# nmonette/TO-UED

Measured on AMD Instinct MI355X. Metric: agent-env-steps/sec (inner rollout) at num_agents=512; meta-updates/sec, higher is better.
Workload: dtype f32; 1 GPU; C2 LPG meta-gradient env_mode=tabular num_agents=512 num_mini_batches=1 W=64 T=20 K=5 score_function=random; num_agents=512, agents_per_gpu=512, env_workers=64, train_rollout_len=20, num_agent_updates=5, parallelism=dp1 (agent axis)

## Files before the change

### to-ued_amd/csrc/gru.hip

```cpp
#include <stdlib.h>
#include <string.h>
#include <algorithm>
#include "common.h"

extern "C" size_t toued_wgrad_workspace_floats(int ra, int rb, long K);
extern "C" int toued_wgrad(int ra, int rb, long K, const float* A, long lda, const float* B, long ldb, float* C,
                           float* work, size_t work_floats, hipStream_t stream);
extern "C" int toued_wgrad_ldc(int ra, int rb, long K, const float* A, long lda, const float* B, long ldb, float* C,
                               int ldc, float* work, size_t work_floats, hipStream_t stream);
extern "C" size_t toued_rowsum_workspace_floats(int ra, long K);
extern "C" int toued_rowsum_into(int ra, long K, const float* A, long lda, float* C, int ldc, float* work,
                                 size_t work_floats, hipStream_t stream);

typedef float floatx16 __attribute__((ext_vector_type(16)));
typedef float floatx4 __attribute__((ext_vector_type(4)));

#define HU 256
#define RB 32
#define LDH 33
#define NAUG 8
#define KQF 33
#define NTILE_F 32

struct EtaOff {
// ... 1211 lines not shown
    }
    __syncthreads();
    float dhn_r[NT][16];
    const float* wil = wi34 + 32 * wave + 4 * hi;
#pragma unroll
    for (int h = 0; h < NT; ++h) {
      floatx16 hacc;
#pragma unroll
      for (int q = 0; q < 16; ++q) hacc[q] = 0.0f;
#pragma unroll
      for (int kk = 0; kk < 5; ++kk) {
        const int o = 2 * kk + hi;
        hacc = mfma32(wA[kk], o < 9 ? hv[o * RBT + RB * h + col] : 0.0f, hacc);
      }
      const unsigned vq = (unsigned)((((long)(32 * wave + 4 * hi + (col & 3))) * p.M + r0 + RB * h + (col & 28)) * 4);
      float dx3 = 0.0f, dx4 = 0.0f;
#pragma unroll
      for (int g4 = 0; g4 < 4; ++g4) {
        const unsigned so = (unsigned)(((long)8 * g4 * p.M + ctr) * 4);
        float v_hin[4], v_r[4], v_z[4], v_n[4], v_hn[4];
        ld4(rs_hin, vq, so, v_hin);
        ld4(rs_r, vq, so, v_r);
        ld4(rs_z, vq, so, v_z);
        ld4(rs_n, vq, so, v_n);
        ld4(rs_hn, vq, so, v_hn);
        quad_transpose(v_hin, lane);
        quad_transpose(v_r, lane);
        quad_transpose(v_z, lane);
        quad_transpose(v_n, lane);
        quad_transpose(v_hn, lane);
        float* o_rh = v_hin; float* o_dr = v_r; float* o_dz = v_z; float* o_dhn = v_n; float* o_dn = v_hn;
#pragma unroll
        for (int j = 0; j < 4; ++j) {
          const int q = 4 * g4 + j;
          const float hin = v_hin[j], rg = v_r[j], zg = v_z[j], ng = v_n[j], hn = v_hn[j];
          const float hout = (1.0f - zg) * ng + zg * hin;
          const float d = dh[h][q] + (hout > 0.0f ? hacc[q] : 0.0f);
          const float dn_ = d * (1.0f - zg);
          const float dz = d * (hin - ng);
          const float dnp = dn_ * (1.0f - ng * ng);
          const float dhn = dnp * rg;
          const float drp = dnp * hn * rg * (1.0f - rg);
          const float dzp = dz * zg * (1.0f - zg);
          dh[h][q] = d * zg;
          const int lo = (32 * wave + 4 * hi + qunit(q)) * LDT + RB * h + col;
          dgT[lo] = drp;
          dgT[HU * LDT + lo] = dzp;
          dhn_r[h][q] = dhn;
          o_rh[j] = fmaxf(hout, 0.0f); o_dr[j] = drp; o_dz[j] = dzp; o_dhn[j] = dhn; o_dn[j] = dnp;
          const int qu = qunit(q);
          dx3 += drp * wil[0 * HU + qu] + dzp * wil[1 * HU + qu] + dnp * wil[2 * HU + qu];
          dx4 += drp * wil[3 * HU + qu] + dzp * wil[4 * HU + qu] + dnp * wil[5 * HU + qu];
        }
        {
          const unsigned vb = (unsigned)(((long)(32 * wave + 4 * hi) * p.M + r0 + RB * h + col) * 4);
#pragma unroll
          for (int j = 0; j < 4; ++j) {
            const unsigned so1 = (unsigned)(((long)qunit(4 * g4 + j) * p.M + ctr) * 4);
            st_u(rs_rh, vb, so1, o_rh[j]);
            st_u(rs_dg[3], vb, so1, o_dn[j]);
          }
        }
      }
      dxp[((2 * wave + hi) * 2 + 0) * RBT + RB * h + col] = dx3;
      dxp[((2 * wave + hi) * 2 + 1) * RBT + RB * h + col] = dx4;
    }
    floatx16 acc[NT];
#pragma unroll
    for (int h = 0; h < NT; ++h)
#pragma unroll
      for (int q = 0; q < 16; ++q) acc[h][q] = 0.0f;
#pragma unroll 1
    for (int g = 0; g < 3; ++g) {
      if (g == 2) {
        __syncthreads();
#pragma unroll
        for (int h = 0; h < NT; ++h) {
          float* dgl = dgT + (32 * wave + 4 * hi) * LDT + RB * h + col;
#pragma unroll
          for (int q = 0; q < 16; ++q) dgl[qunit(q) * LDT] = dhn_r[h][q];
        }
      }
      if (g != 1) __syncthreads();
      if (g == 0) {
        store_gate_lds<NT>(dgT, rs_dg[0], p.M, ctr + r0, wave, lane);
        store_gate_lds<NT>(dgT + HU * LDT, rs_dg[1], p.M, ctr + r0, wave, lane);
      } else if (g == 2) {
        store_gate_lds<NT>(dgT, rs_dg[2], p.M, ctr + r0, wave, lane);
      }
      const float* dgs = dgT + (g == 1 ? HU * LDT : 0);
      float4 an = Ab[((wave * 3 + g) * 32 + 0) * 64];
#pragma unroll 2
      for (int kq = 0; kq < 32; ++kq) {
        const float4 av = an;
        if (kq + 1 < 32) an = Ab[((wave * 3 + g) * 32 + kq + 1) * 64];
#pragma unroll
        for (int e = 0; e < 4; ++e) {
          const float x = e == 0 ? av.x : e == 1 ? av.y : e == 2 ? av.z : av.w;
#pragma unroll
          for (int h = 0; h < NT; ++h) {
            const float b = dgs[(2 * (4 * kq + e) + hi) * LDT + RB * h + col];
            acc[h] = mfma32(x, b, acc[h]);
          }
        }
      }
    }
    __syncthreads();
    if (tid < RBT) {
      float s3 = 0.0f, s4 = 0.0f;
      for (int gq = 0; gq < NGRP; ++gq) { s3 += dxp[(gq * 2 + 0) * RBT + tid]; s4 += dxp[(gq * 2 + 1) * RBT + tid]; }
      p.dX3[ctr + r0 + tid] = s3;
      p.dX4[ctr + r0 + tid] = s4;
    }
#pragma unroll
    for (int h = 0; h < NT; ++h) {
      const bool dn = done[((size_t)a_[h] * T + t) * W + w_[h]] != 0;
#pragma unroll
      for (int q = 0; q < 16; ++q) dh[h][q] = dn ? 0.0f : dh[h][q] + acc[h][q];
    }
    __syncthreads();
  }
}


#ifdef BWD_STAMPS
__device__ unsigned long long g_bwd_stamps[64 * 32 * 8];
#define BWD_STAMP(ph)                                                                                  \
  do {                                                                                                 \
    if (blockIdx.x < 64 && tid == 0 && t < 32)                                                         \
      g_bwd_stamps[(blockIdx.x * 32 + t) * 8 + (ph)] = __builtin_amdgcn_s_memtime();                   \
  } while (0)
#define BWD_NWS 8
__device__ unsigned long long g_bwd_wstamps[64 * 32 * 8 * BWD_NWS];
__device__ int g_bwd_wsimd[64 * 8];
#define BWD_WSTAMP(ph)                                                                                 \
  do {                                                                                                 \
    if (blockIdx.x < 64 && lane_now() == 0 && t < 32)                                                  \
      g_bwd_wstamps[((blockIdx.x * 32 + t) * 8 + wave) * BWD_NWS + (ph)] = __builtin_amdgcn_s_memtime(); \
  } while (0)
#else
#define BWD_STAMP(ph) do {} while (0)
#define BWD_WSTAMP(ph) do {} while (0)
#endif

#ifndef BWD_MPRIO
#define BWD_MPRIO 0
#endif
#ifndef BWD_TRECOMP
#define BWD_TRECOMP 0
#endif
#ifndef BWD_PK
#define BWD_PK 1
#endif
template <bool SMALL>
__global__ void __launch_bounds__(512, 1) k_gru_bwd6n(BwdArgs p) {
  constexpr int RBT = 2 * RB;
  constexpr int PP = HU + 8;
  __shared__ __attribute__((aligned(16))) __bf16 dgB[3][RBT * PP];
  __shared__ float wi34[2 * 3 * HU];
  __shared__ float hv[9 * RBT];
  __shared__ __attribute__((aligned(8))) float dxp[8 * RBT * 2];
  __shared__ __attribute__((aligned(16))) float wsc[HU];
  __shared__ float rmx[8 * RBT];
  __shared__ float wIs[8 * 4 * 64];
  __shared__ float wAs[8 * 5 * 64];
  __shared__ int dns[RBT];
  __shared__ __attribute__((aligned(16))) float Atab[SMALL ? 32 * 64 : 4];
  __shared__ float hvs[SMALL ? 9 * RBT : 1];
  __shared__ floatx4 accl[SMALL ? 8 * 2 * 64 : 1];
  constexpr int DRP = HU + 4;
  static_assert(RBT * DRP * 4 <= 2 * RBT * PP * 2, "dr staging exceeds image slots 1-2");
  float* drs = reinterpret_cast<float*>(&dgB[1][0]);
  const int tid = threadIdx.x, lane = tid & 63, hi = lane >> 5, col = lane & 31;
  const int wave = __builtin_amdgcn_readfirstlane(tid >> 6);
  const int nb = p.R / RBT;
  const int bid = blockIdx.x + p.wg_base;
  const int k = bid / nb;
  const int r0 = (bid - k * nb) * RBT;
  const int R = p.R, T = p.T, W = p.W;
#ifdef BWD_STAMPS
  if (blockIdx.x < 64 && (tid & 63) == 0)
    g_bwd_wsimd[blockIdx.x * 8 + wave] = __builtin_amdgcn_s_getreg((1 << 11) | (4 << 6) | 4);
#endif
  for (int i = tid; i < 2 * 3 * HU; i += 512) {
    const int f = BWD_PK ? 3 + (i & 1) : 3 + i / (3 * HU), g = BWD_PK ? (i >> 1) / HU : (i / HU) % 3,
              u = BWD_PK ? (i >> 1) % HU : i % HU;
    const int base = g == 0 ? p.o.ir_w : g == 1 ? p.o.iz_w : p.o.in_w;
    wi34[i] = f < p.F ? p.eta[base + f * HU + u] : 0.0f;
  }
  for (int i = tid; i < HU; i += 512) wsc[i] = reinterpret_cast<const float*>(p.A6)[B6_SCALES + i];
  const int F = p.F;
  {
    float wI[4];
    load_win_frags(wI, p.eta, p.o, F, wave, lane);
#pragma unroll
    for (int kk = 0; kk < 4; ++kk) wIs[(wave * 4 + kk) * 64 + lane] = wI[kk];
  }
#pragma unroll
  for (int kk = 0; kk < 5; ++kk) {
    const int o = 2 * kk + hi, u = 32 * wave + col;
    wAs[(wave * 5 + kk) * 64 + lane] = o < 9 ? (o == 0 ? p.eta[p.o.pi_w + u] : p.eta[p.o.y_w + u * 8 + (o - 1)]) : 0.0f;
  }
  float dh[2][16];
#pragma unroll
  for (int h = 0; h < 2; ++h)
#pragma unroll
    for (int q = 0; q < 16; ++q) dh[h][q] = 0.0f;
  if (SMALL) {
    for (int i = tid; i < 9 * RBT; i += 512) hvs[i] = 0.0f;
    for (int i = tid; i < 8 * 2 * 64; i += 512) accl[i] = floatx4{0.0f, 0.0f, 0.0f, 0.0f};
  }
  constexpr bool st_rh = !SMALL, st_dn = !SMALL;
  const __amdgpu_buffer_rsrc_t rs_hin = rsrc_of(p.s_hin), rs_r = rsrc_of(p.s_r), rs_z = rsrc_of(p.s_z),
                               rs_hn = rsrc_of(p.s_hn), rs_rh = rsrc_of(SMALL ? p.s_hin : p.RH);
  const __amdgpu_buffer_rsrc_t rs_x = rsrc_of(p.s_hin + (size_t)HU * p.M);
  const __amdgpu_buffer_rsrc_t rs_dg[4] = {rsrc_of(p.DG), rsrc_of(p.DG + 1L * HU * p.M),
                                           rsrc_of(p.DG + 2L * HU * p.M),
                                           rsrc_of(SMALL ? p.DG : p.DG + 3L * HU * p.M)};
  constexpr bool st_DH = !SMALL;
  const __amdgpu_buffer_rsrc_t rs_yh = rsrc_of(p.y_hat), rs_dyh = rsrc_of(p.d_y_hat), rs_dpi = rsrc_of(p.d_pi_hat),
                               rs_DH = rsrc_of(SMALL ? p.dX3 : p.DH), rs_dx3 = rsrc_of(p.dX3), rs_dx4 = rsrc_of(p.dX4),
                               rs_done = rsrc_of(reinterpret_cast<const float*>(p.done + (long)k * p.done_stride_k));
  auto head_cot = [&](int t) {
    if (tid < RBT) {
      const int tl = lane_now();
      const unsigned vrw = (unsigned)tl * 4;
      int dnv;
      {
        const int rw = r0 + tl, a = rw / W;
        dnv = __builtin_amdgcn_raw_buffer_load_b8(rs_done, (a * T + t) * W + rw - a * W, 0, 0);
      }
      const long o = ((long)k * T + t) * R + r0;
      float yh[8], dy[8], s = 0.0f;
#pragma unroll
      for (int j = 0; j < 8; ++j) {
        const unsigned so = (unsigned)((((long)k * T * 8 + (long)t * 8 + j) * R + r0) * 4);
        yh[j] = ld_u(rs_yh, vrw, so);
        dy[j] = ld_u(rs_dyh, vrw, so);
      }
#pragma unroll
      for (int j = 0; j < 8; ++j) s += yh[j] * dy[j];
      const float dpi = ld_u(rs_dpi, vrw, (unsigned)(o * 4));
      float xr[6];
      if (SMALL) {
#pragma unroll
        for (int f = 0; f < 6; ++f)
          xr[f] = ld_u(rs_x, vrw, (unsigned)(((long)(f < F ? f : 0) * p.M + o) * 4));
      }
      dns[tl] = dnv;
      hv[tl] = dpi;
      if (st_DH) st_u(rs_DH, vrw, (unsigned)(o * 4), dpi);
      float hvv[9];
      hvv[0] = dpi;
#pragma unroll
      for (int j = 0; j < 8; ++j) {
        const float v = yh[j] * (dy[j] - s);
        hv[(j + 1) * RBT + tl] = v;
        hvv[j + 1] = v;
        if (st_DH) st_u(rs_DH, vrw, (unsigned)(((long)(j + 1) * p.M + o) * 4), v);
      }
      if (SMALL) {
        float* at = Atab + (tl >> 1) * 64 + 16 * (tl & 1);
#pragma unroll
        for (int c = 0; c < 4; ++c) {
          if (c >= 2) *reinterpret_cast<float4*>(at + 4 * c) = make_float4(0.0f, 0.0f, 0.0f, 0.0f);
          *reinterpret_cast<float4*>(at + 32 + 4 * c) = make_float4(0.0f, 0.0f, 0.0f, 0.0f);
        }
        at[6] = 0.0f;
        at[7] = 0.0f;
        *reinterpret_cast<float4*>(at) = make_float4(0 < F ? xr[0] : 0.0f, 1 < F ? xr[1] : 0.0f, 2 < F ? xr[2] : 0.0f,
                                                     3 < F ? xr[3] : 0.0f);
        *reinterpret_cast<float2*>(at + 4) = make_float2(4 < F ? xr[4] : 0.0f, 5 < F ? xr[5] : 0.0f);
        at[F] = 1.0f;
#pragma unroll
        for (int o9 = 0; o9 < 9; ++o9) at[32 + F + 1 + o9] = hvv[o9];
#pragma unroll
        for (int o9 = 0; o9 < 9; ++o9) hvs[o9 * RBT + tl] += hvv[o9];
      }
    }
  };
  const __amdgpu_buffer_rsrc_t rs_A = rsrc_of(reinterpret_cast<const float*>(p.A6));
  const unsigned vA = (unsigned)lane * 16;
  floatx16 acc[2];
  auto ldAh = [&](int ks, int g, int q) {
    const u32x4 x = __builtin_amdgcn_raw_buffer_load_b128(rs_A, (int)vA,
                                                          (int)((((ks * 8 + wave) * 3 + g) * 3 + q) * 1024), 0);
    return __builtin_bit_cast(f16x8, x);
  };
#ifndef BWD_RD
#define BWD_RD 4
#endif
#ifndef BWD_SPREAD
#define BWD_SPREAD 0
#endif
  auto dg_vbyte = [&](int ub_, int col_) {
    return SMALL ? (unsigned)(ub_ * 128 + col_ * 4) : (unsigned)(((long)ub_ * p.M + r0 + col_) * 4);
  };
  auto dg_soff = [&](long ctr_, int uq, int h) {
    return SMALL ? (unsigned)((((ctr_ + r0) >> 5) + h) * 32768L + uq * 128)
                 : (unsigned)((((long)uq * p.M + ctr_) * 4) + 128 * h);
  };
  auto store_slot = [&](int gst, long ctr_, int gi, int i, float v) {
    const int s_ = 2 * BWD_RD * gi + i, h = s_ >> 4, e = s_ & 3, g4 = (s_ & 15) >> 2;
    const int ln = lane_now();
    st_u(rs_dg[gst], dg_vbyte(32 * wave + 4 * (ln >> 5), ln & 31), dg_soff(ctr_, e + 8 * g4, h), v);
  };
#ifndef BWD_SPLACE
#define BWD_SPLACE 0
#endif
  static_assert(!BWD_SPLACE || (!BWD_SPREAD && 16 % BWD_RD == 0), "BWD_SPLACE: burst stores, RD dividing 16");
  f16x8 ring[BWD_RD][2];
  auto preload_ring = [&](int g) {
#pragma unroll
    for (int i = 0; i < BWD_RD; ++i)
#pragma unroll
      for (int q = 0; q < 2; ++q) ring[i][q] = ldAh(i, g, q);
  };
  auto contract_h = [&](int g, int sb, int sb1, float (&qv)[32], long ctr_, auto&& pre, bool preloaded, int nextg,
                        auto&& post, auto&& inpass) {
    constexpr int RD = BWD_RD;
    static_assert(!BWD_SPREAD || 16 % RD == 0, "the spread stores: 2 per k-step, 2 RD per ring group");
    f16x8 B[2][2];
    if (!preloaded) preload_ring(g);
    const int ln = lane_now(), bl = (ln & 31) * PP + 8 * (ln >> 5);
    auto ldB = [&](int ks, int h) {
#pragma unroll
      for (int q = 0; q < 2; ++q) B[h][q] = *reinterpret_cast<const f16x8*>(&dgB[q ? sb1 : sb][bl + RB * h * PP + 16 * ks]);
    };
    ldB(0, 0);
    ldB(0, 1);
    auto kstep = [&](int ks, f16x8 (&Ar)[2], bool reload, int gi, int j) {
#pragma unroll
      for (int h = 0; h < 2; ++h) {
        acc[h] = mfma3h(Ar, B[h], acc[h]);
        if (ks + 1 < 16) ldB(ks + 1, h);
        if (BWD_SPREAD && h == 0) {
          store_slot(g, ctr_, gi, 2 * j, qv[2 * j]);
          store_slot(g, ctr_, gi, 2 * j + 1, qv[2 * j + 1]);
        }
      }
      if (reload) {
#pragma unroll
        for (int q = 0; q < 2; ++q) Ar[q] = ldAh(ks + RD, g, q);
      }
      __builtin_amdgcn_sched_barrier(0);
    };
    constexpr int NG = (16 - RD) / RD;
#pragma nounroll
    for (int gi = 0; gi < NG; ++gi) {
#pragma unroll
      for (int j = 0; j < RD; ++j) kstep(gi * RD + j, ring[j], true, gi, j);
      if (BWD_SPREAD) {
#pragma unroll
        for (int i = 0; i < 32 - 2 * RD; ++i) qv[i] = qv[i + 2 * RD];
      }
    }
#pragma unroll
    for (int ks = NG * RD; ks < 16; ++ks) {
      kstep(ks, ring[ks % RD], ks + RD < 16, NG, ks - NG * RD);
      if (ks == 16 - RD) {
        pre();
        __builtin_amdgcn_sched_barrier(0);
      }
      if (BWD_SPLACE && nextg >= 0 && ks >= 16 - RD) {
#pragma unroll
        for (int q = 0; q < 2; ++q) ring[ks % RD][q] = ldAh(ks - (16 - RD), nextg, q);
        __builtin_amdgcn_sched_barrier(0);
      }
      if (ks >= 12) {
        inpass(ks - 12);
        __builtin_amdgcn_sched_barrier(0);
      }
    }
    post();
  };
#ifndef BWD_INPASS
#define BWD_INPASS 0
#endif
#ifndef BWD_TREFILL
#define BWD_TREFILL 0
#endif
  auto put4h = [&](int row, int u0, const float (&v)[4], float sc) {
    f16x4 x0, x1;
    if (BWD_TREFILL == 2) {
#pragma unroll
      for (int e = 0; e < 4; ++e) { x0[e] = (_Float16)0.0f; x1[e] = (_Float16)0.0f; }
    } else {
#pragma unroll
      for (int e = 0; e < 4; ++e) split2h(v[e] * sc, x0, x1, e);
    }
    if (BWD_TREFILL != 1) {
      *reinterpret_cast<f16x4*>(&dgB[0][row * PP + u0]) = x0;
      *reinterpret_cast<f16x4*>(&dgB[1][row * PP + u0]) = x1;
    }
  };
  auto put1h = [&](int slot, int which, int row, int u0, const float (&v)[4], float sc) {
    f16x4 x0, x1;
#pragma unroll
    for (int e = 0; e < 4; ++e) split2h(v[e] * sc, x0, x1, e);
    *reinterpret_cast<f16x4*>(&dgB[slot][row * PP + u0]) = which ? x1 : x0;
  };
  float* priv = reinterpret_cast<float*>(&dgB[0][0]) + 1056 * wave;
  auto small_mfma = [&](int h, int g4, const float (&dnq)[4], const float (&rhq)[4]) {
    const int ln = lane_now(), row = ln & 31, c = 2 * (g4 & 1) + (ln >> 5);
    const int wo = row * 16 + ((c ^ ((row >> 2) & 3)) << 2);
    *reinterpret_cast<float4*>(priv + wo) = make_float4(dnq[0], dnq[1], dnq[2], dnq[3]);
    *reinterpret_cast<float4*>(priv + 544 + wo) = make_float4(rhq[0], rhq[1], rhq[2], rhq[3]);
    if (g4 & 1) {
      const int l2 = lane_now(), kk = l2 >> 4, j = l2 & 15;
      const int rb = (kk >> 1) * 544 + (kk & 1) * 16 + (j & 3);
      floatx4& al = accl[(wave * 2 + (g4 >> 1)) * 64 + l2];
      floatx4 acc = al;
#pragma unroll
      for (int s2 = 0; s2 < 16; ++s2) {
        const float b = priv[rb + 32 * s2 + ((((j >> 2) ^ ((s2 >> 1) & 3))) << 2)];
        const float a = Atab[(16 * h + s2) * 64 + l2];
        acc = __builtin_amdgcn_mfma_f32_16x16x4f32(a, b, acc, 0, 0, 0);
      }
      al = acc;
    }
  };
#ifndef BWD_NR
#define BWD_NR 3
#endif
  constexpr int NR = BWD_NR;
  const int ub = 32 * wave + 4 * hi;
  float vr[NR][4][4];
  auto load_q = [&](long ctr_, int h, int g4, float (&v)[4][4]) {
    const unsigned vq = quad_vbyte(ub, col), sq = quad_soff(ctr_ + r0, h, g4);
    if (HIN_SLAB) ld4(rs_hin, slab_vbyte(ub + (col & 3), col & 28), slab_soff(ctr_ + r0, h, 8 * g4), v[0]);
    else ld4(rs_hin, (unsigned)((((long)(ub + (col & 3))) * p.M + r0 + RB * h + (col & 28)) * 4),
             (unsigned)(((long)8 * g4 * p.M + ctr_) * 4), v[0]);
    if (!BWD_TRECOMP) {
      ld4(rs_r, vq, sq, v[1]);
      ld4(rs_z, vq, sq, v[2]);
      ld4(rs_hn, vq, sq, v[3]);
    }
  };
  float xa[4], xb[4];
  auto load_x = [&](long ctr_, int h, float (&x)[4]) {
#pragma unroll
    for (int kk = 0; kk < 4; ++kk) {
      const int ln = lane_now(), k = 2 * kk + (ln >> 5);
      x[kk] = ld_u(rs_x, (unsigned)((((long)(k < F ? k : 0)) * p.M + RB * h + (ln & 31)) * 4), (unsigned)((ctr_ + r0) * 4));
    }
  };
#ifndef BWD_PF
#define BWD_PF 0
#endif
#ifndef BWD_PFX
#define BWD_PFX 0
#endif
  static_assert(BWD_PF >= 0 && BWD_PF <= NR - 1, "BWD_PF: at most the ring's NR - 1 leading quads");
  auto load_first = [&](long ctr_, bool pre) {
    if (pre == (bool)BWD_PFX) load_x(ctr_, 0, xa);
#pragma unroll
    for (int qi = 0; qi < NR - 1; ++qi)
      if (pre == (qi < BWD_PF)) load_q(ctr_, qi >> 2, qi & 3, vr[qi]);
  };
  if (p.stagger > 0 && blockIdx.x < 256) {
    const int ph = p.stagger_mode == 0 ? (blockIdx.x >> 3) & 1 : p.stagger_mode == 1 ? blockIdx.x & 1 : (blockIdx.x >> 3) & 3;
    for (int i = 0; i < ph * p.stagger; ++i) __builtin_amdgcn_s_sleep(127);
  }
  load_first((long)k * T * R, true);
  for (int t = 0; t < T; ++t) {
    const long ctr = ((long)k * T + t) * R;
    BWD_STAMP(0);
    head_cot(t);
    lds_barrier();
    BWD_STAMP(1);
    BWD_WSTAMP(0);
    floatx16 rc[3][2];
    if (BWD_TRECOMP) {
#pragma unroll
      for (int g = 0; g < 3; ++g)
#pragma unroll
        for (int h = 0; h < 2; ++h)
#pragma unroll
          for (int q = 0; q < 16; ++q) rc[g][h][q] = 0.0f;
      f16x8 Ra0[3][2], Ra1[3][2], Rb[2][2];
      const int ln = lane_now(), bl = (ln & 31) * PP + 8 * (ln >> 5);
      auto ldRB = [&](int ks, int h) {
#pragma unroll
        for (int q = 0; q < 2; ++q) Rb[h][q] = *reinterpret_cast<const f16x8*>(&dgB[q][bl + RB * h * PP + 16 * ks]);
      };
#pragma unroll
      for (int g = 0; g < 3; ++g)
#pragma unroll
        for (int q = 0; q < 2; ++q) {
          Ra0[g][q] = ldAh(0, g, q);
          Ra1[g][q] = ldAh(1, g, q);
        }
      ldRB(0, 0);
      ldRB(0, 1);
      auto rstep = [&](int ks, f16x8 (&Ar)[3][2], bool reload) {
#pragma unroll
        for (int g = 0; g < 3; ++g) {
#pragma unroll
          for (int h = 0; h < 2; ++h) {
            rc[g][h] = mfma3h(Ar[g], Rb[h], rc[g][h]);
            if (g == 2 && ks + 1 < 16) ldRB(ks + 1, h);
          }
          if (reload) {
#pragma unroll
            for (int q = 0; q < 2; ++q) Ar[g][q] = ldAh(ks + 2, g, q);
          }
          __builtin_amdgcn_sched_barrier(0);
        }
      };
#pragma nounroll
      for (int kp = 0; kp < 7; ++kp) {
        rstep(2 * kp, Ra0, true);
        rstep(2 * kp + 1, Ra1, true);
      }
      rstep(14, Ra0, false);
      rstep(15, Ra1, false);
      lds_barrier();
    }
    float dz_r[2][16], dhn_r[2][16];
    auto ubn = [&] { return 32 * wave + 4 * (lane_now() >> 5); };
    auto rown = [&](int h) { return RB * h + (lane_now() & 31); };
    auto st_q = [&](__amdgpu_buffer_rsrc_t rs, int h, int g4, const float (&v)[4]) {
#pragma unroll
      for (int e = 0; e < 4; ++e)
        st_u(rs, (unsigned)(((long)ub * p.M + r0 + RB * h + col) * 4),
             (unsigned)(((long)qunit(4 * g4 + e) * p.M + ctr) * 4), v[e]);
    };
    load_first(ctr, false);
    floatx16 ain;
    floatx16 hacc;
    float dx3 = 0.0f, dx4 = 0.0f;
    float rmr[2] = {0.0f, 0.0f};
#pragma unroll
    for (int qi = 0; qi < 8; ++qi) {
      const int h = qi >> 2, g4 = qi & 3;
      if (BWD_MPRIO == 1) {
        if (((qi + (wave >> 2)) & 1) == 0) __builtin_amdgcn_s_setprio(2); else __builtin_amdgcn_s_setprio(1);
      } else if (BWD_MPRIO == 2 && qi == 0) {
        if (wave >= 4) __builtin_amdgcn_s_setprio(2); else __builtin_amdgcn_s_setprio(1);
      }
      float (&v)[4][4] = vr[qi % NR];
      if (qi + NR - 1 < 8) load_q(ctr, (qi + NR - 1) >> 2, (qi + NR - 1) & 3, vr[(qi + NR - 1) % NR]);
      if (qi == 3) load_x(ctr, 1, xb);
      __builtin_amdgcn_sched_barrier(0);
      if (g4 == 0) {
#pragma unroll
        for (int q = 0; q < 16; ++q) hacc[q] = 0.0f;
#pragma unroll
        for (int kk = 0; kk < 5; ++kk) {
          const int ln = lane_now(), o = 2 * kk + (ln >> 5);
          hacc = mfma32(wAs[(wave * 5 + kk) * 64 + ln], o < 9 ? hv[o * RBT + RB * h + (ln & 31)] : 0.0f, hacc);
        }
        float wI[4];
#pragma unroll
        for (int kk = 0; kk < 4; ++kk) wI[kk] = wIs[(wave * 4 + kk) * 64 + lane];
        ain = gate_ain(wI, F, hi, [&](int k) { return h ? xb[k >> 1] : xa[k >> 1]; });
        dx3 = 0.0f;
        dx4 = 0.0f;
      }
      quad_transpose(v[0], lane);
      const float* wil = wi34 + ubn();
      float drq[4], rhq[4], dnq[4];
      if (BWD_PK) {
        const f2v* wil2 = reinterpret_cast<const f2v*>(wi34) + ubn();
        f2v dx34 = {dx3, dx4};
#pragma unroll
        for (int pp = 0; pp < 2; ++pp) {
          const int j0 = 2 * pp, q0 = 4 * g4 + j0;
          const f2v hin = {v[0][j0], v[0][j0 + 1]}, rg = {v[1][j0], v[1][j0 + 1]}, zg = {v[2][j0], v[2][j0 + 1]},
                    hn = {v[3][j0], v[3][j0 + 1]};
          const f2v ng = {gate_n(ain[q0], rg.x, hn.x), gate_n(ain[q0 + 1], rg.y, hn.y)};
          const f2v omz = 1.0f - zg;
          const f2v hout = omz * ng + zg * hin;
          const f2v hac = {hout.x > 0.0f ? hacc[q0] : 0.0f, hout.y > 0.0f ? hacc[q0 + 1] : 0.0f};
          const f2v d = f2v{dh[h][q0], dh[h][q0 + 1]} + hac;
          const f2v dn_ = d * omz;
          const f2v dz = d * (hin - ng);
          const f2v dnp = dn_ * (1.0f - ng * ng);
          const f2v dhn = dnp * rg;
          const f2v drp = dnp * hn * rg * (1.0f - rg);
          const f2v dzp = dz * zg * omz;
          const f2v dhv = d * zg;
#pragma unroll
          for (int e = 0; e < 2; ++e) {
            const int q = q0 + e, qu = qunit(q);
            dh[h][q] = dhv[e];
            drq[j0 + e] = drp[e];
            dz_r[h][q] = dzp[e];
            dhn_r[h][q] = dhn[e];
            rhq[j0 + e] = fmaxf(hout[e], 0.0f);
            dnq[j0 + e] = dnp[e];
            dx34 += f2v{drp[e], drp[e]} * wil2[0 * HU + qu] + f2v{dzp[e], dzp[e]} * wil2[1 * HU + qu] +
                    f2v{dnp[e], dnp[e]} * wil2[2 * HU + qu];
          }
        }
        dx3 = dx34.x;
        dx4 = dx34.y;
      }
#pragma unroll
      for (int jj = 0; jj < (BWD_PK ? 0 : 4); ++jj) {
        const int q = 4 * g4 + jj;
        const float hin = v[0][jj];
        const float rg = BWD_TRECOMP ? sigm_r(rc[0][h][q] * 0.5f) : v[1][jj];
        const float zg = BWD_TRECOMP ? sigm_r(rc[1][h][q] * 0.5f) : v[2][jj];
        const float hn = BWD_TRECOMP ? rc[2][h][q] * 0.5f : v[3][jj];
        const float ng = gate_n(ain[q], rg, hn);
        const float hout = (1.0f - zg) * ng + zg * hin;
        const float d = dh[h][q] + (hout > 0.0f ? hacc[q] : 0.0f);
        const float dn_ = d * (1.0f - zg);
        const float dz = d * (hin - ng);
        const float dnp = dn_ * (1.0f - ng * ng);
        const float dhn = dnp * rg;
        const float drp = dnp * hn * rg * (1.0f - rg);
        const float dzp = dz * zg * (1.0f - zg);
        dh[h][q] = d * zg;
        drq[jj] = drp;
        dz_r[h][q] = dzp;
        dhn_r[h][q] = dhn;
        const int qu = qunit(q);
        dx3 += drp * wil[0 * HU + qu] + dzp * wil[1 * HU + qu] + dnp * wil[2 * HU + qu];
        dx4 += drp * wil[3 * HU + qu] + dzp * wil[4 * HU + qu] + dnp * wil[5 * HU + qu];
        rhq[jj] = fmaxf(hout, 0.0f);
        dnq[jj] = dnp;
      }
      if (st_rh) st_q(rs_rh, h, g4, rhq);
      if (st_dn) st_q(rs_dg[3], h, g4, dnq);
      if (SMALL) small_mfma(h, g4, dnq, rhq);
      *reinterpret_cast<float4*>(&drs[rown(h) * DRP + ubn() + 8 * g4]) = make_float4(drq[0], drq[1], drq[2], drq[3]);
#pragma unroll
      for (int jj = 0; jj < 4; ++jj) rmr[h] = fmaxf(rmr[h], fabsf(drq[jj]));
      if (g4 == 3) {
        const float f3 = dx3 + __shfl_xor(dx3, 32), f4 = dx4 + __shfl_xor(dx4, 32);
        const int ln = lane_now();
        if (ln < 32) *reinterpret_cast<float2*>(dxp + (wave * RBT + RB * h + ln) * 2) = make_float2(f3, f4);
      }
      __builtin_amdgcn_sched_barrier(0);
    }
    if (BWD_MPRIO) __builtin_amdgcn_s_setprio(0);
    BWD_STAMP(2);
    BWD_WSTAMP(1);
#pragma unroll
    for (int h = 0; h < 2; ++h) {
      float m = rmr[h];
#pragma unroll
      for (int q = 0; q < 16; ++q) m = fmaxf(m, fmaxf(fabsf(dz_r[h][q]), fabsf(dhn_r[h][q])));
      m = fmaxf(m, __shfl_xor(m, 32));
      const int ln = lane_now();
      if (ln < 32) rmx[wave * RBT + RB * h + ln] = m;
    }
    lds_barrier();
    BWD_STAMP(3);
    float bs[2];
#pragma unroll
    for (int h = 0; h < 2; ++h) {
      float m = 0.0f;
      const int cl = lane_now() & 31;
#pragma unroll
      for (int w8 = 0; w8 < 8; ++w8) m = fmaxf(m, rmx[w8 * RBT + RB * h + cl]);
      int sc = 0, ce = 127;
      if (m > 0.0f && m <= 3.0e38f) {
        int e;
        frexpf(m, &e);
        sc = min(40, max(-40, 14 - e));
        ce = min(126, max(-126, 14 - e));
      }
      bs[h] = ldexpf(1.0f, sc);
      if (p.CE && wave == 0 && lane_now() < 32) p.CE[ctr + r0 + rown(h)] = (int8_t)ce;
    }
    auto store_dg = [&](int g, int row, int g4, const float (&v)[4]) {
#pragma unroll
      for (int e = 0; e < 4; ++e)
        st_u(rs_dg[g], dg_vbyte(ub, col), dg_soff(ctr, qunit(4 * g4 + e), row >= RB ? 1 : 0), v[e]);
    };
    float qv[32];
    if (BWD_SPLACE) preload_ring(0);
    {
      f16x4 x1h[2][4];
#pragma unroll
      for (int h = 0; h < 2; ++h)
#pragma unroll
        for (int g4 = 0; g4 < 4; ++g4) {
          const int row = rown(h), un = ubn();
          const float4 v = *reinterpret_cast<const float4*>(&drs[row * DRP + un + 8 * g4]);
          const float v4[4] = {v.x, v.y, v.z, v.w};
          f16x4 x0;
#pragma unroll
          for (int e = 0; e < 4; ++e) split2h(v4[e] * bs[h], x0, x1h[h][g4], e);
          *reinterpret_cast<f16x4*>(&dgB[0][row * PP + un + 8 * g4]) = x0;
          if (BWD_SPREAD) {
#pragma unroll
            for (int e = 0; e < 4; ++e) qv[16 * h + 4 * g4 + e] = v4[e];
          } else {
            store_dg(0, RB * h, g4, v4);
          }
        }
      lds_barrier();
#pragma unroll
      for (int h = 0; h < 2; ++h)
#pragma unroll
        for (int g4 = 0; g4 < 4; ++g4)
          *reinterpret_cast<f16x4*>(&dgB[1][rown(h) * PP + ubn() + 8 * g4]) = x1h[h][g4];
      lds_barrier();
    }
    const int un0 = ubn();
#pragma unroll
    for (int g4 = 0; g4 < 4; ++g4) {
      const float4 w4 = *reinterpret_cast<const float4*>(&wsc[un0 + 8 * g4]);
      const float wv[4] = {w4.x, w4.y, w4.z, w4.w};
#pragma unroll
      for (int h = 0; h < 2; ++h)
#pragma unroll
        for (int e = 0; e < 4; ++e) acc[h][4 * g4 + e] = dh[h][4 * g4 + e] * (wv[e] * bs[h]);
    }
    BWD_STAMP(4);
    BWD_WSTAMP(2);
    auto inpass_put = [&](int j, int slot, const float (&src)[2][16]) {
#pragma unroll
      for (int i = 2 * j; i < 2 * j + 2; ++i) {
        const int h = i >> 2, g4 = i & 3;
        const float v4[4] = {src[h][4 * g4], src[h][4 * g4 + 1], src[h][4 * g4 + 2], src[h][4 * g4 + 3]};
        put1h(slot, 0, rown(h), ubn() + 8 * g4, v4, bs[h]);
      }
    };
    contract_h(0, 0, 1, qv, ctr, [] {}, (bool)BWD_SPLACE, BWD_SPLACE ? 1 : -1, [&] {
      if (BWD_SPLACE) {
#pragma unroll
        for (int h = 0; h < 2; ++h)
#pragma unroll
          for (int g4 = 0; g4 < 4; ++g4) {
            const float v4[4] = {dz_r[h][4 * g4], dz_r[h][4 * g4 + 1], dz_r[h][4 * g4 + 2], dz_r[h][4 * g4 + 3]};
            store_dg(1, RB * h, g4, v4);
          }
      }
    }, [&](int j) {
      if (BWD_INPASS) inpass_put(j, 2, dz_r);
    });
    BWD_WSTAMP(3);
    lds_barrier();
    BWD_WSTAMP(4);
#pragma unroll
    for (int h = 0; h < 2; ++h)
#pragma unroll
      for (int g4 = 0; g4 < 4; ++g4) {
        const float v4[4] = {dz_r[h][4 * g4], dz_r[h][4 * g4 + 1], dz_r[h][4 * g4 + 2], dz_r[h][4 * g4 + 3]};
        if (BWD_INPASS) put1h(0, 1, rown(h), ubn() + 8 * g4, v4, bs[h]);
        else put4h(rown(h), ubn() + 8 * g4, v4, bs[h]);
        if (BWD_SPREAD) {
#pragma unroll
          for (int e = 0; e < 4; ++e) qv[16 * h + 4 * g4 + e] = v4[e];
        } else if (!BWD_SPLACE) {
          store_dg(1, RB * h, g4, v4);
        }
      }
    lds_barrier();
    BWD_STAMP(5);
    BWD_WSTAMP(5);
    contract_h(1, BWD_INPASS ? 2 : 0, BWD_INPASS ? 0 : 1, qv, ctr, [] {}, (bool)BWD_SPLACE, BWD_SPLACE ? 2 : -1, [&] {
      if (BWD_SPLACE) {
#pragma unroll
        for (int h = 0; h < 2; ++h)
#pragma unroll
          for (int g4 = 0; g4 < 4; ++g4) {
            const float v4[4] = {dhn_r[h][4 * g4], dhn_r[h][4 * g4 + 1], dhn_r[h][4 * g4 + 2], dhn_r[h][4 * g4 + 3]};
            store_dg(2, RB * h, g4, v4);
          }
      }
    }, [&](int j) {
      if (BWD_INPASS) inpass_put(j, 1, dhn_r);
    });
    BWD_WSTAMP(6);
    lds_barrier();
    BWD_WSTAMP(7);
#pragma unroll
    for (int h = 0; h < 2; ++h)
#pragma unroll
      for (int g4 = 0; g4 < 4; ++g4) {
        const float v4[4] = {dhn_r[h][4 * g4], dhn_r[h][4 * g4 + 1], dhn_r[h][4 * g4 + 2], dhn_r[h][4 * g4 + 3]};
        if (BWD_INPASS) put1h(2, 1, rown(h), ubn() + 8 * g4, v4, bs[h]);
        else put4h(rown(h), ubn() + 8 * g4, v4, bs[h]);
        if (BWD_SPREAD) {
#pragma unroll
          for (int e = 0; e < 4; ++e) qv[16 * h + 4 * g4 + e] = v4[e];
        } else if (!BWD_SPLACE) {
          store_dg(2, RB * h, g4, v4);
        }
      }
    lds_barrier();
    BWD_STAMP(6);
    contract_h(2, BWD_INPASS ? 1 : 0, BWD_INPASS ? 2 : 1, qv, ctr, [&] {
      if (t + 1 < T) load_first(ctr + R, true);
    }, (bool)BWD_SPLACE, -1, [] {}, [](int) {});
#pragma unroll
    for (int g4 = 0; g4 < 4; ++g4) {
      const float4 w4 = *reinterpret_cast<const float4*>(&wsc[32 * wave + 4 * (lane_now() >> 5) + 8 * g4]);
      const float wv[4] = {w4.x, w4.y, w4.z, w4.w};
#pragma unroll
      for (int h = 0; h < 2; ++h)
#pragma unroll
        for (int e = 0; e < 4; ++e) acc[h][4 * g4 + e] *= inv_pow2(wv[e] * bs[h]);
    }
    if (tid < RBT) {
      const int tl = lane_now();
      float s3 = 0.0f, s4 = 0.0f;
#pragma unroll
      for (int w8 = 0; w8 < 8; ++w8) {
        const float2 v = *reinterpret_cast<const float2*>(dxp + (w8 * RBT + tl) * 2);
        s3 += v.x;
        s4 += v.y;
      }
      st_u(rs_dx3, (unsigned)tl * 4, (unsigned)((ctr + r0) * 4), s3);
      st_u(rs_dx4, (unsigned)tl * 4, (unsigned)((ctr + r0) * 4), s4);
    }
#pragma unroll
    for (int h = 0; h < 2; ++h) {
      const bool dn = dns[RB * h + (lane_now() & 31)] != 0;
#pragma unroll
      for (int q = 0; q < 16; ++q) dh[h][q] = dn ? 0.0f : acc[h][q];
    }
    BWD_STAMP(7);
    lds_barrier();
  }
  if (SMALL) {
    float* out = p.SP + (size_t)bid * SP_FLOATS;
    const int ln = lane_now();
#pragma unroll
    for (int uh = 0; uh < 2; ++uh) {
      const floatx4 a = accl[(wave * 2 + uh) * 64 + ln];
#pragma unroll
      for (int r = 0; r < 4; ++r) out[(4 * (ln >> 4) + r) * HU + 32 * wave + 16 * uh + (ln & 15)] = a[r];
    }
    for (int i = tid; i < 9 * RBT; i += 512) out[SP_C + i] = hvs[i];
  }
}

__global__ void k_sleep_quanta(int q) {
  for (int i = 0; i < q; ++i) __builtin_amdgcn_s_sleep(127);
}

#define SR_CHUNK 64
__global__ void __launch_bounds__(256) k_small_part(const float* __restrict__ sp, int n_wg, float* __restrict__ part2) {
  const int o = blockIdx.x * 256 + threadIdx.x;
  if (o >= SP_FLOATS) return;
  const int c = blockIdx.y, w0 = c * SR_CHUNK, w1 = min(n_wg, w0 + SR_CHUNK);
  float a = 0.0f;
  for (int w = w0; w < w1; ++w) a += sp[(size_t)w * SP_FLOATS + o];
  part2[(size_t)c * SP_FLOATS + o] = a;
}
__global__ void __launch_bounds__(256) k_small_final(const float* __restrict__ part2, int n_chunk, int F,
                                                     float* __restrict__ GI) {
  const int o = blockIdx.x * 256 + threadIdx.x;
  if (o >= 8 * HU + 9 * (HU + 1)) return;
  float a = 0.0f;
  if (o < 8 * HU) {
    const int i = o / HU, u = o % HU;
    if (i <= F)
      for (int c = 0; c < n_chunk; ++c) a += part2[(size_t)c * SP_FLOATS + i * HU + u];
  } else {
    const int e = o - 8 * HU, oo = e / (HU + 1), u = e % (HU + 1);
    if (u < HU) {
      for (int c = 0; c < n_chunk; ++c) a += part2[(size_t)c * SP_FLOATS + (F + 1 + oo) * HU + u];
    } else {
      for (int c = 0; c < n_chunk; ++c) {
        float rs = 0.0f;
        for (int r = 0; r < 64; ++r) rs += part2[(size_t)c * SP_FLOATS + SP_C + oo * 64 + r];
        a += rs;
      }
    }
  }
  GI[o] = a;
}

}

extern "C" {

int toued_gru_pack(const float* eta, const int* off, int F, float* fwdA, float* bwdA, hipStream_t stream) {
  TOUED_REQUIRE(F >= 1 && F <= 7, "toued_gru_pack: F=%d", F);
  EtaOff o;
  memcpy(&o, off, sizeof(EtaOff));
  const int n1 = NTILE_F * KQF * 64, n2 = 8 * 3 * 32 * 64, n3 = F6_NGRP * 64;
  hipLaunchKernelGGL(k_pack_fwd, dim3((n1 + 255) / 256), dim3(256), 0, stream, eta, o, F,
                     reinterpret_cast<float4*>(fwdA), 0L, 0L);
  hipLaunchKernelGGL(k_fwd6_scales, dim3(16), dim3(256), 0, stream, eta, o, fwdA + (size_t)n1 * 4 + F6_SCALES, 0L, 0L);
  hipLaunchKernelGGL(k_pack_fwd6, dim3((n3 + 255) / 256), dim3(256), 0, stream, eta, o, F,
                     reinterpret_cast<bf16x8*>(fwdA + (size_t)n1 * 4), 0L, 0L);
  hipLaunchKernelGGL(k_pack_bwd, dim3((n2 + 255) / 256), dim3(256), 0, stream, eta, o,
                     reinterpret_cast<float4*>(bwdA));
  hipLaunchKernelGGL(k_bwd6_scales, dim3(HU / 4), dim3(256), 0, stream, eta, o, bwdA + (size_t)n2 * 4 + B6_SCALES);
  hipLaunchKernelGGL(k_pack_bwd6, dim3((16 * 8 * 3 * 64 + 255) / 256), dim3(256), 0, stream, eta, o,
                     reinterpret_cast<__bf16*>(bwdA + (size_t)n2 * 4));
  TOUED_CHECK_LAUNCH();
  return 0;
}

size_t toued_gru_packed_floats(int which) {
  const size_t f32_part = (size_t)NTILE_F * KQF * 64 * 4;
  return which == 1 ? (size_t)8 * 3 * 32 * 64 * 4 + B6_FLOATS : f32_part + F6_FLOATS;
}

static bool gru_f32_forced() {
  static const bool f = [] {
    const char* e = getenv("TOUED_GRU_F32");
    return e && e[0] == '1';
  }();
  return f;
}

static int gru_fwd_launch(int R, int T, int W, int F, const float* X, long xs_f, long xs_col, const uint8_t* done,
                          const float* fwdA, const float* eta, const int* off, float* pi_hat, float* y_hat,
                          float* s_hin, float* s_r, float* s_z, float* s_n, float* s_hn, long M, int save, int rpc,
                          long eta_stride, hipStream_t stream) {
  FwdArgs p;
  p.R = R; p.T = T; p.W = W; p.F = F; p.X = X; p.xs_f = xs_f; p.xs_col = xs_col; p.done = done;
  p.A = reinterpret_cast<const float4*>(fwdA); p.eta = eta;
  p.A6 = fwdA + (size_t)NTILE_F * KQF * 64 * 4;
  memcpy(&p.o, off, sizeof(EtaOff));
  p.pi_hat = pi_hat; p.y_hat = y_hat; p.s_hin = s_hin; p.s_r = s_r; p.s_z = s_z; p.s_n = s_n; p.s_hn = s_hn; p.M = M;
  p.rpc = rpc; p.a_stride4 = (long)toued_gru_packed_floats(2) / 4; p.eta_stride = eta_stride;
  static const int stagger = getenv("TOUED_FWD_STAGGER") ? atoi(getenv("TOUED_FWD_STAGGER")) : 3;
  static const int stagger_save = getenv("TOUED_FWD_STAGGER_SAVE") ? atoi(getenv("TOUED_FWD_STAGGER_SAVE")) : 0;
  p.stagger = save ? stagger_save : stagger;
  const bool nt2 = R % (2 * RB) == 0 && (rpc == 0 || rpc % (2 * RB) == 0);
  if (nt2 && !gru_f32_forced()) {
    if (save) hipLaunchKernelGGL(k_gru_fwd6<true>, dim3(R / (2 * RB)), dim3(512), 0, stream, p);
    else hipLaunchKernelGGL(k_gru_fwd6<false>, dim3(R / (2 * RB)), dim3(512), 0, stream, p);
  } else if (save) {
    if (nt2) hipLaunchKernelGGL((k_gru_fwd<true, 2>), dim3(R / (2 * RB)), dim3(512), 0, stream, p);
    else hipLaunchKernelGGL((k_gru_fwd<true, 1>), dim3(R / RB), dim3(512), 0, stream, p);
  } else {
    if (nt2) hipLaunchKernelGGL((k_gru_fwd<false, 2>), dim3(R / (2 * RB)), dim3(512), 0, stream, p);
    else hipLaunchKernelGGL((k_gru_fwd<false, 1>), dim3(R / RB), dim3(512), 0, stream, p);
  }
  TOUED_CHECK_LAUNCH();
  return 0;
}

int toued_gru_fwd(int R, int T, int W, int F, const float* X, long xs_f, long xs_col, const uint8_t* done,
                  const float* fwdA, const float* eta, const int* off, float* pi_hat, float* y_hat, float* s_hin,
                  float* s_r, float* s_z, float* s_n, float* s_hn, long M, hipStream_t stream) {
  TOUED_REQUIRE(R % RB == 0 && W % RB == 0, "toued_gru_fwd: rows R=%d and workers W=%d must be multiples of 32", R, W);
  TOUED_REQUIRE(F >= 1 && F <= 7 && T >= 1, "toued_gru_fwd: F=%d T=%d", F, T);
  TOUED_REQUIRE((double)M * 264.0 * 4.0 < 4294967295.0, "toued_gru_fwd: M=%ld columns exceed the 4 GiB buffer range "
                "(use --num_mini_batches to split the agent batch)", M);
  TOUED_REQUIRE(s_hin && s_r && s_z && s_n && s_hn, "toued_gru_fwd: saved-activation buffers required");
  return gru_fwd_launch(R, T, W, F, X, xs_f, xs_col, done, fwdA, eta, off, pi_hat, y_hat, s_hin, s_r, s_z, s_n, s_hn,
                        M, 1, 0, 0, stream);
}

int toued_gru_pack_fwd_multi(const float* eta, long eta_stride, int n, const int* off, int F, float* fwdA,
                             hipStream_t stream) {
  TOUED_REQUIRE(F >= 1 && F <= 7 && n >= 0, "toued_gru_pack_fwd_multi: F=%d n=%d", F, n);
  if (n == 0) return 0;
  EtaOff o;
  memcpy(&o, off, sizeof(EtaOff));
  const int n1 = NTILE_F * KQF * 64;
  const long cstride = (long)toued_gru_packed_floats(2);
  hipLaunchKernelGGL(k_pack_fwd, dim3((n1 + 255) / 256, n), dim3(256), 0, stream, eta, o, F,
                     reinterpret_cast<float4*>(fwdA), eta_stride, cstride / 4);
  const int n3 = F6_NGRP * 64;
  hipLaunchKernelGGL(k_fwd6_scales, dim3(16, n), dim3(256), 0, stream, eta, o, fwdA + (size_t)n1 * 4 + F6_SCALES,
                     eta_stride, cstride);
  hipLaunchKernelGGL(k_pack_fwd6, dim3((n3 + 255) / 256, n), dim3(256), 0, stream, eta, o, F,
                     reinterpret_cast<bf16x8*>(fwdA + (size_t)n1 * 4), eta_stride, cstride / 4);
  TOUED_CHECK_LAUNCH();
  return 0;
}

int toued_gru_fwd_multi(int R, int T, int W, int F, int rows_per_cand, const float* X, long xs_f, long xs_col,
                        const uint8_t* done, const float* fwdA, const float* eta, long eta_stride, const int* off,
                        float* pi_hat, float* y_hat, hipStream_t stream) {
  TOUED_REQUIRE(R % RB == 0 && W % RB == 0, "toued_gru_fwd_multi: rows R=%d and workers W=%d must be multiples of 32",
                R, W);
  TOUED_REQUIRE(rows_per_cand > 0 && rows_per_cand % RB == 0 && R % rows_per_cand == 0,
                "toued_gru_fwd_multi: rows_per_cand=%d must be a multiple of 32 dividing R=%d", rows_per_cand, R);
  TOUED_REQUIRE(F >= 1 && F <= 7 && T >= 1, "toued_gru_fwd_multi: F=%d T=%d", F, T);
  return gru_fwd_launch(R, T, W, F, X, xs_f, xs_col, done, fwdA, eta, off, pi_hat, y_hat, nullptr, nullptr, nullptr,
                        nullptr, nullptr, 0, 0, rows_per_cand, eta_stride, stream);
}

int toued_gru_bwd_col_exp(int R) { return R % (2 * RB) == 0 && !gru_f32_forced() ? 1 : 0; }

int toued_gru_bwd(int R, int T, int W, int K, const uint8_t* done, long done_stride_k, const float* bwdA,
                  const float* eta, const int* off, const float* y_hat, const float* d_pi_hat, const float* d_y_hat,
                  const float* s_hin, const float* s_r, const float* s_z, const float* s_n, const float* s_hn, long M,
                  float* DG, float* RH, float* DH, float* dX3, float* dX4, int8_t* col_exp, hipStream_t stream) {
  TOUED_REQUIRE(R % RB == 0 && W % RB == 0, "toued_gru_bwd: rows R=%d and workers W=%d must be multiples of 32", R, W);
// ... 147 lines not shown
```

Baseline: 182.4 million agent-env-steps/sec.

## Software-pipeline GRU backward head cotangent loads across timesteps

Splits the per-timestep head cotangent computation into a load phase and a put phase. The next timestep's loads are issued inside the previous step's contraction, and their results are written to LDS at the end of that step. This removes one barrier and the load latency at the start of each timestep. The done flags are double-buffered in LDS by timestep parity, and the first-quad prefetch for the next step now happens unconditionally right after the contraction. The cost is extra live registers for the prefetched head values, which may raise register pressure in a kernel launched with one block of 512 threads.

```diff
diff --git a/to-ued_amd/csrc/gru.hip b/to-ued_amd/csrc/gru.hip
--- a/to-ued_amd/csrc/gru.hip
+++ b/to-ued_amd/csrc/gru.hip
@@ -1387,6 +1387,12 @@
 #ifndef BWD_PK
 #define BWD_PK 1
 #endif
+#ifndef BWD_HEADPIPE
+#define BWD_HEADPIPE 1
+#endif
+#ifndef BWD_LOADTOP
+#define BWD_LOADTOP 1
+#endif
 template <bool SMALL>
 __global__ void __launch_bounds__(512, 1) k_gru_bwd6n(BwdArgs p) {
   constexpr int RBT = 2 * RB;
@@ -1399,7 +1405,7 @@
   __shared__ float rmx[8 * RBT];
   __shared__ float wIs[8 * 4 * 64];
   __shared__ float wAs[8 * 5 * 64];
-  __shared__ int dns[RBT];
+  __shared__ int dns[(BWD_HEADPIPE ? 2 : 1) * RBT];
   __shared__ __attribute__((aligned(16))) float Atab[SMALL ? 32 * 64 : 4];
   __shared__ float hvs[SMALL ? 9 * RBT : 1];
   __shared__ floatx4 accl[SMALL ? 8 * 2 * 64 : 1];
@@ -1453,36 +1459,49 @@
                                            rsrc_of(p.DG + 2L * HU * p.M),
                                            rsrc_of(SMALL ? p.DG : p.DG + 3L * HU * p.M)};
   constexpr bool st_DH = !SMALL;
+  const __amdgpu_buffer_rsrc_t rs_DH = rsrc_of(SMALL ? p.dX3 : p.DH), rs_dx3 = rsrc_of(p.dX3), rs_dx4 = rsrc_of(p.dX4);
   const __amdgpu_buffer_rsrc_t rs_yh = rsrc_of(p.y_hat), rs_dyh = rsrc_of(p.d_y_hat), rs_dpi = rsrc_of(p.d_pi_hat),
-                               rs_DH = rsrc_of(SMALL ? p.dX3 : p.DH), rs_dx3 = rsrc_of(p.dX3), rs_dx4 = rsrc_of(p.dX4),
                                rs_done = rsrc_of(reinterpret_cast<const float*>(p.done + (long)k * p.done_stride_k));
-  auto head_cot = [&](int t) {
-    if (tid < RBT) {
+#define HEAD_IN_DECL float hd_yh[8], hd_dy[8], hd_dpi, hd_xr[6]; int hd_dnv
+#define HEAD_IN hd_yh, hd_dy, hd_dpi, hd_xr, hd_dnv
+  auto head_load = [&](int t, float (&yh)[8], float (&dy)[8], float& dpi, float (&xr)[6], int& dnv) {
+#pragma unroll
+    for (int j = 0; j < 8; ++j) yh[j] = dy[j] = 0.0f;
+#pragma unroll
+    for (int f = 0; f < 6; ++f) xr[f] = 0.0f;
+    dpi = 0.0f;
+    dnv = 0;
+    if (wave == 0) {
       const int tl = lane_now();
       const unsigned vrw = (unsigned)tl * 4;
-      int dnv;
       {
         const int rw = r0 + tl, a = rw / W;
         dnv = __builtin_amdgcn_raw_buffer_load_b8(rs_done, (a * T + t) * W + rw - a * W, 0, 0);
       }
       const long o = ((long)k * T + t) * R + r0;
-      float yh[8], dy[8], s = 0.0f;
 #pragma unroll
       for (int j = 0; j < 8; ++j) {
         const unsigned so = (unsigned)((((long)k * T * 8 + (long)t * 8 + j) * R + r0) * 4);
         yh[j] = ld_u(rs_yh, vrw, so);
         dy[j] = ld_u(rs_dyh, vrw, so);
       }
-#pragma unroll
-      for (int j = 0; j < 8; ++j) s += yh[j] * dy[j];
-      const float dpi = ld_u(rs_dpi, vrw, (unsigned)(o * 4));
-      float xr[6];
+      dpi = ld_u(rs_dpi, vrw, (unsigned)(o * 4));
       if (SMALL) {
 #pragma unroll
         for (int f = 0; f < 6; ++f)
           xr[f] = ld_u(rs_x, vrw, (unsigned)(((long)(f < F ? f : 0) * p.M + o) * 4));
       }
-      dns[tl] = dnv;
+    }
+  };
+  auto head_put = [&](int t, const float (&yh)[8], const float (&dy)[8], float dpi, const float (&xr)[6], int dnv) {
+    if (wave == 0) {
+      const int tl = lane_now();
+      const unsigned vrw = (unsigned)tl * 4;
+      const long o = ((long)k * T + t) * R + r0;
+      float s = 0.0f;
+#pragma unroll
+      for (int j = 0; j < 8; ++j) s += yh[j] * dy[j];
+      dns[(BWD_HEADPIPE ? (t & 1) * RBT : 0) + tl] = dnv;
       hv[tl] = dpi;
       if (st_DH) st_u(rs_DH, vrw, (unsigned)(o * 4), dpi);
       float hvv[9];
@@ -1680,30 +1699,34 @@
       x[kk] = ld_u(rs_x, (unsigned)((((long)(k < F ? k : 0)) * p.M + RB * h + (ln & 31)) * 4), (unsigned)((ctr_ + r0) * 4));
     }
   };
-#ifndef BWD_PF
-#define BWD_PF 0
-#endif
-#ifndef BWD_PFX
-#define BWD_PFX 0
-#endif
-  static_assert(BWD_PF >= 0 && BWD_PF <= NR - 1, "BWD_PF: at most the ring's NR - 1 leading quads");
-  auto load_first = [&](long ctr_, bool pre) {
-    if (pre == (bool)BWD_PFX) load_x(ctr_, 0, xa);
-#pragma unroll
-    for (int qi = 0; qi < NR - 1; ++qi)
-      if (pre == (qi < BWD_PF)) load_q(ctr_, qi >> 2, qi & 3, vr[qi]);
+  auto load_first = [&](long ctr_) {
+    load_x(ctr_, 0, xa);
+#pragma unroll
+    for (int qi = 0; qi < NR - 1; ++qi) load_q(ctr_, qi >> 2, qi & 3, vr[qi]);
   };
   if (p.stagger > 0 && blockIdx.x < 256) {
     const int ph = p.stagger_mode == 0 ? (blockIdx.x >> 3) & 1 : p.stagger_mode == 1 ? blockIdx.x & 1 : (blockIdx.x >> 3) & 3;
     for (int i = 0; i < ph * p.stagger; ++i) __builtin_amdgcn_s_sleep(127);
   }
-  load_first((long)k * T * R, true);
+  if (BWD_HEADPIPE) {
+    HEAD_IN_DECL;
+    head_load(0, HEAD_IN);
+    head_put(0, HEAD_IN);
+    if (BWD_LOADTOP) load_first((long)k * T * R);
+    lds_barrier();
+  } else if (BWD_LOADTOP) {
+    load_first((long)k * T * R);
+  }
   for (int t = 0; t < T; ++t) {
     const long ctr = ((long)k * T + t) * R;
     BWD_STAMP(0);
-    head_cot(t);
-    lds_barrier();
-    BWD_STAMP(1);
+    HEAD_IN_DECL;
+    if (!BWD_HEADPIPE) {
+      head_load(t, HEAD_IN);
+      head_put(t, HEAD_IN);
+      lds_barrier();
+      BWD_STAMP(1);
+    }
     BWD_WSTAMP(0);
     floatx16 rc[3][2];
     if (BWD_TRECOMP) {
@@ -1761,7 +1784,7 @@
         st_u(rs, (unsigned)(((long)ub * p.M + r0 + RB * h + col) * 4),
              (unsigned)(((long)qunit(4 * g4 + e) * p.M + ctr) * 4), v[e]);
     };
-    load_first(ctr, false);
+    if (!BWD_LOADTOP) load_first(ctr);
     floatx16 ain;
     floatx16 hacc;
     float dx3 = 0.0f, dx4 = 0.0f;
@@ -2023,8 +2046,10 @@
     lds_barrier();
     BWD_STAMP(6);
     contract_h(2, BWD_INPASS ? 1 : 0, BWD_INPASS ? 2 : 1, qv, ctr, [&] {
-      if (t + 1 < T) load_first(ctr + R, true);
+      if (BWD_HEADPIPE) head_load(min(t + 1, T - 1), HEAD_IN);
     }, (bool)BWD_SPLACE, -1, [] {}, [](int) {});
+    if (BWD_HEADPIPE) BWD_STAMP(1);
+    if (BWD_LOADTOP) load_first(t + 1 < T ? ctr + R : ctr);
 #pragma unroll
     for (int g4 = 0; g4 < 4; ++g4) {
       const float4 w4 = *reinterpret_cast<const float4*>(&wsc[32 * wave + 4 * (lane_now() >> 5) + 8 * g4]);
@@ -2048,10 +2073,11 @@
     }
 #pragma unroll
     for (int h = 0; h < 2; ++h) {
-      const bool dn = dns[RB * h + (lane_now() & 31)] != 0;
+      const bool dn = dns[(BWD_HEADPIPE ? (t & 1) * RBT : 0) + RB * h + (lane_now() & 31)] != 0;
 #pragma unroll
       for (int q = 0; q < 16; ++q) dh[h][q] = dn ? 0.0f : acc[h][q];
     }
+    if (BWD_HEADPIPE && t + 1 < T) head_put(t + 1, HEAD_IN);
     BWD_STAMP(7);
     lds_barrier();
   }
@@ -2067,6 +2093,9 @@
     for (int i = tid; i < 9 * RBT; i += 512) out[SP_C + i] = hvs[i];
   }
 }
+
+#undef HEAD_IN_DECL
+#undef HEAD_IN
 
 __global__ void k_sleep_quanta(int q) {
   for (int i = 0; i < q; ++i) __builtin_amdgcn_s_sleep(127);
```

After: 183.7 million agent-env-steps/sec (median of 6 runs). Within noise of the previous version (+0.7%).
